# cubefs/cubefs

Measured on AMD Instinct MI355X. Metric: GiB/s encode+CRC throughput, RS(k+m) per stripe, 1/2/4/8 MI355X vs CPU, higher is better.
Workload: dtype u8; 1 GPU; RS(6+3) fused encode+frame, 8 MiB shards, 1024 stripes/GPU; codemode=EC6P3, stripes_per_gpu=1024, crc_included=True, block_len=65536

## Files before the change

### cubefs_amd/csrc/gfrs_kernels.hip

```cpp
#include "gfrs_internal.h"

#include <cstdio>
#include <cstdlib>
#include <type_traits>

namespace gfrs {

static int env_grid(const char *name, int dflt) {
  const char *v = getenv(name);
  if (!v) return dflt;
  int x = atoi(v);
  return x > 0 ? x : dflt;
}

typedef uint32_t u32x4 __attribute__((ext_vector_type(4)));

static bool nt_enabled() {
  static int v = -1;
  if (v < 0) {
    const char *e = getenv("GFRS_NT");
    v = e ? (atoi(e) != 0) : 0;
  }
  return v == 1;
}
// ... 532 lines not shown
                     hipStream_t s) {
  ShardAddr a{ptrs, 0, 0, nptr};
  rs_dispatch<false>(a, in_idx, k, out_idx, nout, tabs, shard_len, nstripes,
                     nullptr, s);
}

void launch_rs_apply_strided(uint64_t base, uint64_t stripe_stride,
                             const int32_t *in_idx, int k,
                             const int32_t *out_idx, int nout,
                             const uint8_t *tabs, size_t shard_len,
                             int nstripes, hipStream_t s) {
  ShardAddr a{nullptr, base, stripe_stride, 0};
  rs_dispatch<false>(a, in_idx, k, out_idx, nout, tabs, shard_len, nstripes,
                     nullptr, s);
}

void launch_rs_verify(const uint64_t *ptrs, int nptr, const int32_t *in_idx,
                      int k, const int32_t *out_idx, int nout,
                      const uint8_t *tabs, size_t shard_len, int nstripes,
                      uint32_t *fail, hipStream_t s) {
  ShardAddr a{ptrs, 0, 0, nptr};
  rs_dispatch<true>(a, in_idx, k, out_idx, nout, tabs, shard_len, nstripes,
                    fail, s);
}

void launch_rs_verify_strided(uint64_t base, uint64_t stripe_stride,
                              const int32_t *in_idx, int k,
                              const int32_t *out_idx, int nout,
                              const uint8_t *tabs, size_t shard_len,
                              int nstripes, uint32_t *fail, hipStream_t s) {
  ShardAddr a{nullptr, base, stripe_stride, 0};
  rs_dispatch<true>(a, in_idx, k, out_idx, nout, tabs, shard_len, nstripes,
                    fail, s);
}


__global__ void probe_perm_k(uint32_t *out) {
  if (threadIdx.x == 0) {
    out[0] = __builtin_amdgcn_perm(0x44332211u, 0x88776655u, 0x03020100u);
    out[1] = __builtin_amdgcn_perm(0x44332211u, 0x88776655u, 0x07060504u);
    out[2] = __builtin_amdgcn_perm(0xAABBCCDDu, 0x11223344u, 0x0B0A0908u);
    out[3] = __builtin_amdgcn_perm(0xAABBCCDDu, 0x11223344u, 0x0F0E0D0Cu);
    out[4] = __builtin_amdgcn_perm(0x80808080u, 0x7F7F7F7Fu, 0x0B0A0908u);
  }
}

static int g_perm0 = -1;

int probe_perm_device(void) {
  uint32_t *d = nullptr;
  uint32_t h[5] = {1, 1, 1, 1, 1};
  if (hipMalloc(&d, sizeof(h)) != hipSuccess) return -100;
  hipLaunchKernelGGL(probe_perm_k, dim3(1), dim3(64), 0, nullptr, d);
  if (hipMemcpy(h, d, sizeof(h), hipMemcpyDeviceToHost) != hipSuccess) {
    hipFree(d);
    return -100;
  }
  hipFree(d);
  const bool order_ok = (h[0] == 0x88776655u) && (h[1] == 0x44332211u);
  if (!order_ok) return -103;
  fprintf(stderr,
          "gfrs perm probe: sel8-11(lo=0x11223344,hi=0xAABBCCDD)=%08x "
          "sel12-15=%08x sel8-11(sign)=%08x\n", h[2], h[3], h[4]);
  g_perm0 = (h[2] == 0u) ? 1 : 0;
  return g_perm0;
}

static bool perm0_ok() {
  if (g_perm0 < 0) {
    int r = probe_perm_device();
    if (r < 0) g_perm0 = 0;
  }
  return g_perm0 == 1;
}


#define CRC_POLY 0xEDB88320u
#define CRC_LEN 4

__device__ uint32_t g_crc_tab4[8][256];
__device__ uint32_t g_shift4k[4][256];
__device__ uint32_t g_shift1k[4][256];
__device__ uint32_t g_shift8k[4][256];

__device__ uint32_t g_pow8[40];

GFRS_DEV int64_t i64min(int64_t a, int64_t b) { return a < b ? a : b; }

GFRS_DEV uint32_t gf2_mulmod_d(uint32_t a, uint32_t b) {
  uint32_t prod = 0;
#pragma unroll 8
  for (int i = 31; i >= 0; i--) {
    if ((a >> i) & 1) prod ^= b;
    b = (b & 1) ? (b >> 1) ^ CRC_POLY : (b >> 1);
  }
  return prod;
}

GFRS_DEV uint32_t x8n_d(uint64_t len) {
  uint32_t op = 0x80000000u;
  int j = 0;
  while (len) {
    if (len & 1) op = gf2_mulmod_d(op, g_pow8[j]);
    len >>= 1;
    j++;
  }
  return op;
}

constexpr int CRC_BLOCKT = 256;

GFRS_DEV uint32_t xor3(uint32_t a, uint32_t b, uint32_t c) {
  return __builtin_amdgcn_bitop3_b32(a, b, c, 0x96);
}

GFRS_DEV uint32_t crc16_reg(const uint4 q, const uint32_t (*tab)[256]) {
  uint32_t c = 0;
#pragma unroll
  for (int j = 0; j < 2; j++) {
    const uint32_t w0 = (j == 0 ? q.x : q.z) ^ c;
    const uint32_t w1 = (j == 0 ? q.y : q.w);
    c = xor3(xor3(tab[7][w0 & 0xFF], tab[6][(w0 >> 8) & 0xFF],
                  tab[5][(w0 >> 16) & 0xFF]),
             xor3(tab[4][w0 >> 24], tab[3][w1 & 0xFF],
                  tab[2][(w1 >> 8) & 0xFF]),
             tab[1][(w1 >> 16) & 0xFF] ^ tab[0][w1 >> 24]);
  }
  return c;
}

GFRS_DEV uint32_t shift4k(uint32_t c, const uint32_t (*stab)[256]) {
  return xor3(stab[0][c & 0xFF], stab[1][(c >> 8) & 0xFF],
              stab[2][(c >> 16) & 0xFF]) ^
         stab[3][c >> 24];
}

GFRS_DEV uint32_t crc_chunk(const uint8_t *p, int len,
                            const uint32_t (*tab)[256], uint8_t *dst) {
  uint32_t c = 0;
  int i = 0;
  for (; i + 4 <= len; i += 4) {
    const uint32_t w = *reinterpret_cast<const uint32_t *>(p + i);
    if (dst) *reinterpret_cast<uint32_t *>(dst + i) = w;
    c ^= w;
    c = tab[3][c & 0xFF] ^ tab[2][(c >> 8) & 0xFF] ^ tab[1][(c >> 16) & 0xFF] ^
        tab[0][c >> 24];
  }
  for (; i < len; i++) {
    if (dst) dst[i] = p[i];
    c = tab[0][(c ^ p[i]) & 0xFF] ^ (c >> 8);
  }
  return c;
}

GFRS_DEV uint32_t crc_chunk16(const uint8_t *p, int len,
                              const uint32_t (*tab)[256]) {
  uint32_t c = 0;
  int i = 0;
  for (; i + 16 <= len; i += 16) {
    const uint4 q = *reinterpret_cast<const uint4 *>(p + i);
#pragma unroll
    for (int j = 0; j < 2; j++) {
      const uint32_t w0 = (j == 0 ? q.x : q.z) ^ c;
      const uint32_t w1 = (j == 0 ? q.y : q.w);
      c = xor3(xor3(tab[7][w0 & 0xFF], tab[6][(w0 >> 8) & 0xFF],
                    tab[5][(w0 >> 16) & 0xFF]),
// ... 1071 lines not shown
              const uint8_t b = tailb[c2 * 16 + (p - t0)];
              pv ^= gfmul1_lin(ctab + size_t(r * k + c2) * 32, b);
            }
            fdst[p] = pv;
            part ^= gf2_mulmod_d(x8tab[rbi - 1 - p], tab[0][pv]);
          }
        }
#pragma unroll
        for (int sh = 32; sh > 0; sh >>= 1)
          part ^= __shfl_xor(part, sh, 64);
        if ((threadIdx.x & 63) == 0)
          red[(threadIdx.x >> 6) * 16 + k + r] ^= part;
      }
    }

    __syncthreads();
    {
      const int j = int(threadIdx.x);
      if (j < k + GM) {
        const uint32_t it =
            payload == payload_full
                ? it_full
                : gf2_mulmod_d(x8n_d(uint64_t(payload)), 0xFFFFFFFFu);
        const uint32_t crc =
            ~(it ^ red[j] ^ red[16 + j] ^ red[32 + j] ^ red[48 + j]);
        *reinterpret_cast<uint32_t *>(
            dst + (stripe * (k + GM) + j) * dst_stride + f * block_len) = crc;
      }
    }
    if (tiny_len && f == frames_per_shard - 1) {
      const int j = int(threadIdx.x);
      const int64_t tp0 = (f + 1) * payload_full;
      if (j < k) {
        const uint8_t *sp = sbase + size_t(j) * shard_len + tp0;
        for (int b = 0; b < tiny_len; b++) tinyb[j * 64 + b] = sp[b];
      }
      __syncthreads();
      if (j < k + GM) {
        uint8_t *tb =
            dst + (stripe * (k + GM) + j) * dst_stride + (f + 1) * block_len;
        uint32_t cr = 0;
        for (int b = 0; b < tiny_len; b++) {
          uint8_t x;
          if (j < k) {
            x = tinyb[j * 64 + b];
          } else {
            x = 0;
            for (int c2 = 0; c2 < k; c2++)
              x ^= gfmul1_lin(ctab + size_t((j - k) * k + c2) * 32,
                              tinyb[c2 * 64 + b]);
          }
          tb[CRC_LEN + b] = x;
          cr = tab[0][(cr ^ x) & 0xFF] ^ (cr >> 8);
        }
        *reinterpret_cast<uint32_t *>(tb) =
            ~(gf2_mulmod_d(x8n_d(uint64_t(tiny_len)), 0xFFFFFFFFu) ^ cr);
      }
    }
    __syncthreads();
  }
}



typedef uint32_t u32x3a __attribute__((ext_vector_type(3)));
struct AlLd {
  uint4 v[4];
  u32x3a e;
};

template <bool FULL>
GFRS_DEV AlLd al_load(const uint8_t *sp, int r, int P, int nfull, int q0) {
  AlLd o;
#pragma unroll
  for (int i = 0; i < 4; i++) {
    const int q = q0 + 64 * i;
    const bool lm = FULL ? (i > 0 || q > 0 || r < 3)
                         : (q <= nfull && 16 * q - 4 - 4 * r < P &&
                            16 * q + 12 - 4 * r > 0);
    o.v[i] = lm ? *reinterpret_cast<const uint4 *>(sp + 16 * q)
                : uint4{0, 0, 0, 0};
  }
  const int qe = q0 + 193;
  const bool em = (threadIdx.x & 63) == 63 && r > 0 &&
                  (FULL || (qe <= nfull && 16 * qe - 4 - 4 * r < P));
  o.e = em ? *reinterpret_cast<const u32x3a *>(sp + 16 * qe)
           : u32x3a{0, 0, 0};
  return o;
}

GFRS_DEV uint32_t al_shl1(uint32_t edge, uint32_t own) {
  return uint32_t(__builtin_amdgcn_update_dpp(int(edge), int(own),
                                              0x130 , 0xF,
                                              0xF, false));
}
GFRS_DEV uint32_t al_rol1(uint32_t v) {
  return uint32_t(__builtin_amdgcn_update_dpp(0, int(v),
                                              0x134 , 0xF,
                                              0xF, false));
}

GFRS_DEV uint32_t al_mulmod(uint32_t a, uint32_t b) {
  uint32_t prod = 0;
#pragma unroll
  for (int i = 31; i >= 0; i--) {
    const uint32_t ma = uint32_t(int32_t(a << (31 - i)) >> 31);
    prod ^= b & ma;
    const uint32_t mb = uint32_t(int32_t(b << 31) >> 31);
    b = (b >> 1) ^ (CRC_POLY & mb);
  }
  return prod;
}

GFRS_DEV uint32_t al_wave_xor(uint32_t x) {
  x ^= uint32_t(__builtin_amdgcn_update_dpp(0, int(x), 0xB1 , 0xF, 0xF, true));
  x ^= uint32_t(__builtin_amdgcn_update_dpp(0, int(x), 0x4E , 0xF, 0xF, true));
  x ^= uint32_t(__builtin_amdgcn_update_dpp(0, int(x),
                                            0x141 , 0xF,
                                            0xF, true));
  x ^= uint32_t(__builtin_amdgcn_update_dpp(0, int(x), 0x140 ,
                                            0xF, 0xF, true));
  return uint32_t(__builtin_amdgcn_readlane(int(x), 0) ^
                  __builtin_amdgcn_readlane(int(x), 16) ^
                  __builtin_amdgcn_readlane(int(x), 32) ^
                  __builtin_amdgcn_readlane(int(x), 48));
}

template <int R>
GFRS_DEV void al_rot(uint4 (&d)[4], const AlLd &c) {
#pragma unroll
  for (int i = 0; i < 4; i++) {
    const uint4 own = c.v[i];
    uint32_t n[3] = {0, 0, 0};
#pragma unroll
    for (int j = 0; j < R; j++) {
      const uint32_t ownj = j == 0 ? own.x : j == 1 ? own.y : own.z;
      uint32_t edge;
      if (i < 3) {
        const uint4 nx = c.v[i < 3 ? i + 1 : 3];
        edge = al_rol1(j == 0 ? nx.x : j == 1 ? nx.y : nx.z);
      } else {
        edge = j == 0 ? c.e.x : j == 1 ? c.e.y : c.e.z;
      }
      n[j] = al_shl1(edge, ownj);
    }
    d[i] = R == 0   ? own
           : R == 1 ? uint4{own.y, own.z, own.w, n[0]}
           : R == 2 ? uint4{own.z, own.w, n[0], n[1]}
                    : uint4{own.w, n[0], n[1], n[2]};
  }
}

template <int GM, int WPS, int SKEL = 0, int ST = 0, int C0 = 0>
__global__ __launch_bounds__(CRC_BLOCKT, WPS) void rs_encode_frame_al_k(
    uint8_t *__restrict__ dst, size_t dst_stride, uint64_t base,
    uint64_t stripe_stride, size_t shard_len, int k,
    const uint8_t *__restrict__ tabs , int64_t total_frames,
    int64_t frames_per_shard, int tiny_len ) {
  constexpr int64_t block_len = 65536;
  constexpr int payload_full = 65532;
  extern __shared__ __attribute__((aligned(16))) unsigned char smem[];
  uint32_t(*tab)[256] = reinterpret_cast<uint32_t(*)[256]>(smem);
  uint32_t(*stab)[256] = reinterpret_cast<uint32_t(*)[256]>(smem + 8192);
  uint32_t *red = reinterpret_cast<uint32_t *>(smem + 12288);
  uint32_t *x8tab = reinterpret_cast<uint32_t *>(smem + 12288 + EF_RED);
  uint8_t *tailb = smem + 12288 + EF_RED + 64;
  uint8_t *tinyb = smem + 12288 + EF_RED + 64 + 256;
  uint32_t *c0b =
      reinterpret_cast<uint32_t *>(smem + 12288 + EF_RED + 64 + 256 + 1024);
  uint8_t *ctab = smem + 12288 + EF_RED + 64 + 256 + 1024 + 256;
  for (int i = threadIdx.x; i < 2048; i += CRC_BLOCKT)
    (&tab[0][0])[i] = (&g_crc_tab4[0][0])[i];
  for (int i = threadIdx.x; i < 1024; i += CRC_BLOCKT)
    (&stab[0][0])[i] = (&g_shift1k[0][0])[i];
  for (int i = threadIdx.x; i < GM * k * 2; i += CRC_BLOCKT)
    reinterpret_cast<uint4 *>(ctab)[i] =
        reinterpret_cast<const uint4 *>(tabs)[i];
  if (threadIdx.x == 0) {
    uint32_t v = 0x80000000u;
    for (int j = 0; j < 16; j++) {
      x8tab[j] = v;
      v = gf2_mulmod_d(v, g_pow8[0]);
    }
  }
  const int tid = int(threadIdx.x);
  const int ql0 = (tid >> 6) * 256 + (tid & 63);
  constexpr uint32_t INV16K = 0x479933FCu;
  const uint32_t op_pA = x8n_d(uint64_t(65536 - 16 * (ql0 + 192 + 1)));
  const uint32_t op_pB = gf2_mulmod_d(op_pA, INV16K);
  const uint32_t op_pC = gf2_mulmod_d(op_pB, INV16K);
  const uint32_t op_pD = gf2_mulmod_d(op_pC, INV16K);
  const uint32_t it_full =
      gf2_mulmod_d(x8n_d(uint64_t(payload_full)), 0xFFFFFFFFu);
  __syncthreads();

  const int64_t fr0 = blockIdx.x, frS = gridDim.x;
  int64_t stripe = fr0 / frames_per_shard;
  int64_t f = fr0 - stripe * frames_per_shard;
  const int64_t dstripe = frS / frames_per_shard;
  const int64_t drem = frS - dstripe * frames_per_shard;
  AlLd nx = {};
  if (fr0 < total_frames) {
    const int64_t p0 = f * payload_full;
    const int r = int((3 * f + 3) & 3);
    const int P = int(i64min(payload_full, int64_t(shard_len) - p0));
    nx = al_load<false>(
        as_global(base + stripe * stripe_stride) + (p0 - 4 - 4 * r), r, P,
        (P + 4) >> 4, ql0);
  }
  for (int64_t fr = fr0; fr < total_frames; fr += frS) {
    int64_t stripe2 = stripe + dstripe, f2 = f + drem;
    if (f2 >= frames_per_shard) {
      f2 -= frames_per_shard;
      ++stripe2;
    }
    const int64_t p0 = f * payload_full;
    const int r = int((3 * f + 3) & 3);
    const int P = int(i64min(payload_full, int64_t(shard_len) - p0));
    const int T = P + 4;
    const int nfull = T >> 4;
    const int tb = T & 15;
    const int ntot = (T + 15) >> 4;
    const int64_t abase = p0 - 4 - 4 * r;
    const uint8_t *sbase = as_global(base + stripe * stripe_stride);

    for (int j = threadIdx.x; j < 64; j += CRC_BLOCKT) red[j] = 0;
    __syncthreads();

    auto passes = [&](auto fullc) {
    constexpr bool FULL = decltype(fullc)::value;
    uint4 acc[GM][4];
    for (int h = 0; h < 4; h++) {
      if (!FULL && 1024 * h >= ntot) break;
      const int qp = 1024 * h + ql0;
      const bool tail = !FULL && tb != 0 && (nfull >> 10) == h;
#pragma unroll
      for (int rr = 0; rr < GM; rr++)
#pragma unroll
        for (int i = 0; i < 4; i++) acc[rr][i] = uint4{0, 0, 0, 0};

      uint32_t op = h == 0   ? op_pA
                    : h == 1 ? op_pB
                    : h == 2 ? op_pC
                             : op_pD;
      if (!FULL) {
        int np = 0;
#pragma unroll
        for (int i = 0; i < 4; i++)
          if (qp + 64 * i < nfull) np = i + 1;
        const int end = np ? 16 * (qp + 64 * (np - 1) + 1) : 0;
        op = x8n_d(uint64_t(T - end));
      }

      for (int c = 0; c < k; c++) {
        const uint8_t *src = sbase + size_t(c) * shard_len;
        uint8_t *fdst =
            dst + (stripe * (k + GM) + c) * dst_stride + f * block_len;
        LinTab lt[GM];
        if (SKEL != 1)
#pragma unroll
          for (int rr = 0; rr < GM; rr++)
            lt[rr] = lintab_load(ctab, rr * k + c);
        const AlLd cur = nx;
        if (c + 1 < k)
          nx = al_load<FULL>(src + shard_len + abase, r, P, nfull, qp);
        uint4 d[4];
        switch (r) {
          case 0: al_rot<0>(d, cur); break;
          case 1: al_rot<1>(d, cur); break;
          case 2: al_rot<2>(d, cur); break;
          default: al_rot<3>(d, cur); break;
        }
        if (qp == 0) d[0].x = 0;
        uint32_t t = 0;
#pragma unroll
        for (int i = 0; i < 4; i++) {
          const int q = qp + 64 * i;
          if (FULL || q < nfull) {
            const uint4 v = d[i];
            if (SKEL != 1) {
#pragma unroll
              for (int dd = 0; dd < 4; dd++)
                gfmac4_lin_rows<GM>(acc, i, dd, (&v.x)[dd], lt);
            }
            if (i == 0 && q == 0) {
              if (C0 == 0) {
                *reinterpret_cast<u32x3a *>(fdst + 4) =
                    u32x3a{v.y, v.z, v.w};
              } else {
                c0b[c * 4 + 1] = v.y;
                c0b[c * 4 + 2] = v.z;
                c0b[c * 4 + 3] = v.w;
              }
            } else {
              fstore16<ST>(fdst + 16 * q, v);
            }
            if (SKEL != 1) t = shift4k(t, stab) ^ crc16_reg(v, tab);
          }
        }
        uint32_t part = al_mulmod(op, t);
        if (tail) {
          const int p = 16 * nfull + tid;
          if (p < T) {
            const uint8_t x = src[p0 + p - 4];
            fdst[p] = x;
            tailb[c * 16 + tid] = x;
            if (SKEL != 1)
              part ^= gf2_mulmod_d(x8tab[T - 1 - p], tab[0][x]);
          }
        }
        part = al_wave_xor(part);
        if ((tid & 63) == 0) red[(tid >> 6) * 16 + c] ^= part;
      }
      if (tail) __syncthreads();
      {
        if (FULL ? h < 3 : 1024 * (h + 1) < ntot) {
          nx = al_load<FULL>(sbase + abase, r, P, nfull, qp + 1024);
        } else if (fr + frS < total_frames) {
          const int64_t p02 = f2 * payload_full;
          const int r2 = int((3 * f2 + 3) & 3);
          const int P2 = int(i64min(payload_full, int64_t(shard_len) - p02));
          nx = al_load<false>(as_global(base + stripe2 * stripe_stride) +
                                  (p02 - 4 - 4 * r2),
                              r2, P2, (P2 + 4) >> 4, ql0);
        }
      }
#pragma unroll
      for (int rr = 0; rr < GM; rr++) {
        uint8_t *fdst =
            dst + (stripe * (k + GM) + k + rr) * dst_stride + f * block_len;
        uint32_t t = 0;
#pragma unroll
        for (int i = 0; i < 4; i++) {
          const int q = qp + 64 * i;
          if (FULL || q < nfull) {
            const uint4 v = acc[rr][i];
            if (i == 0 && q == 0) {
              if (C0 == 0) {
                *reinterpret_cast<u32x3a *>(fdst + 4) =
                    u32x3a{v.y, v.z, v.w};
              } else {
                c0b[(k + rr) * 4 + 1] = v.y;
                c0b[(k + rr) * 4 + 2] = v.z;
                c0b[(k + rr) * 4 + 3] = v.w;
              }
            } else {
              fstore16<ST>(fdst + 16 * q, v);
            }
            if (SKEL != 1) t = shift4k(t, stab) ^ crc16_reg(v, tab);
          }
        }
        uint32_t part = al_mulmod(op, t);
        if (SKEL != 1 && tail) {
          const int p = 16 * nfull + tid;
          if (p < T) {
            uint8_t pv = 0;
            for (int c2 = 0; c2 < k; c2++) {
              const uint8_t b = tailb[c2 * 16 + tid];
              pv ^= gfmul1_lin(ctab + size_t(rr * k + c2) * 32, b);
            }
            fdst[p] = pv;
            part ^= gf2_mulmod_d(x8tab[T - 1 - p], tab[0][pv]);
          }
        }
        part = al_wave_xor(part);
        if ((tid & 63) == 0) red[(tid >> 6) * 16 + k + rr] ^= part;
      }
    }
    };
    if (P == payload_full)
      passes(std::true_type{});
    else
      passes(std::false_type{});

    __syncthreads();
    {
      const int j = tid;
      if (j < k + GM) {
        const uint32_t it =
            P == payload_full
                ? it_full
                : gf2_mulmod_d(x8n_d(uint64_t(P)), 0xFFFFFFFFu);
        const uint32_t crc =
            ~(it ^ red[j] ^ red[16 + j] ^ red[32 + j] ^ red[48 + j]);
        uint8_t *fb0 =
            dst + (stripe * (k + GM) + j) * dst_stride + f * block_len;
        if (C0 == 1 && nfull > 0)
          *reinterpret_cast<uint4 *>(fb0) =
              uint4{crc, c0b[j * 4 + 1], c0b[j * 4 + 2], c0b[j * 4 + 3]};
        else
          *reinterpret_cast<uint32_t *>(fb0) = crc;
      }
    }
    if (tiny_len && f == frames_per_shard - 1) {
      const int j = tid;
      const int64_t tp0 = (f + 1) * payload_full;
      if (j < k) {
        const uint8_t *sp = sbase + size_t(j) * shard_len + tp0;
        for (int b = 0; b < tiny_len; b++) tinyb[j * 64 + b] = sp[b];
      }
      __syncthreads();
      if (j < k + GM) {
        uint8_t *tb2 =
            dst + (stripe * (k + GM) + j) * dst_stride + (f + 1) * block_len;
        uint32_t cr = 0;
        for (int b = 0; b < tiny_len; b++) {
          uint8_t x;
          if (j < k) {
            x = tinyb[j * 64 + b];
          } else {
            x = 0;
            for (int c2 = 0; c2 < k; c2++)
              x ^= gfmul1_lin(ctab + size_t((j - k) * k + c2) * 32,
                              tinyb[c2 * 64 + b]);
          }
          tb2[CRC_LEN + b] = x;
          cr = tab[0][(cr ^ x) & 0xFF] ^ (cr >> 8);
        }
        *reinterpret_cast<uint32_t *>(tb2) =
            ~(gf2_mulmod_d(x8n_d(uint64_t(tiny_len)), 0xFFFFFFFFu) ^ cr);
      }
    }
    __syncthreads();
    stripe = stripe2;
    f = f2;
  }
}




GFRS_DEV uint32_t crc_dw(uint32_t c, uint32_t w, const uint32_t (*tab)[256]) {
  c ^= w;
  return tab[3][c & 0xFF] ^ tab[2][(c >> 8) & 0xFF] ^
         tab[1][(c >> 16) & 0xFF] ^ tab[0][c >> 24];
}

GFRS_DEV uint32_t shift8k(uint32_t c, const uint32_t (*stab)[256]) {
  return xor3(stab[0][c & 0xFF], stab[1][(c >> 8) & 0xFF],
              stab[2][(c >> 16) & 0xFF]) ^
         stab[3][c >> 24];
}

GFRS_DEV uint32_t crc32_reg(const uint4 qa, const uint4 qb,
                            const uint32_t (*tab)[256]) {
  uint32_t c = 0;
#pragma unroll
  for (int j = 0; j < 4; j++) {
    const uint32_t w0 =
        (j == 0 ? qa.x : j == 1 ? qa.z : j == 2 ? qb.x : qb.z) ^ c;
    const uint32_t w1 = (j == 0 ? qa.y : j == 1 ? qa.w : j == 2 ? qb.y : qb.w);
    c = xor3(xor3(tab[7][w0 & 0xFF], tab[6][(w0 >> 8) & 0xFF],
                  tab[5][(w0 >> 16) & 0xFF]),
             xor3(tab[4][w0 >> 24], tab[3][w1 & 0xFF],
                  tab[2][(w1 >> 8) & 0xFF]),
             tab[1][(w1 >> 16) & 0xFF] ^ tab[0][w1 >> 24]);
  }
  return c;
}

typedef uint32_t u32x3_t __attribute__((ext_vector_type(3)));
template <int D0>
GFRS_DEV void rot_tail_load(uint4 &w2, const uint8_t *p) {
  if (D0 == 1) {
    w2.x = *reinterpret_cast<const uint32_t *>(p);
  } else if (D0 == 2) {
    const uint2 t = *reinterpret_cast<const uint2 *>(p);
    w2.x = t.x;
    w2.y = t.y;
  } else if (D0 == 3) {
    const u32x3_t t = *reinterpret_cast<const u32x3_t *>(p);
    w2.x = t.x;
    w2.y = t.y;
    w2.z = t.z;
  }
}

template <int D0>
GFRS_DEV void rot_pick(uint4 &h0, uint4 &h1, const uint4 w0, const uint4 w1,
                       const uint4 w2) {
  const uint32_t a[12] = {w0.x, w0.y, w0.z, w0.w, w1.x, w1.y,
                          w1.z, w1.w, w2.x, w2.y, w2.z, w2.w};
  h0 = uint4{a[D0], a[D0 + 1], a[D0 + 2], a[D0 + 3]};
  h1 = uint4{a[D0 + 4], a[D0 + 5], a[D0 + 6], a[D0 + 7]};
}

struct RotArgs {
  uint8_t *dst;
  const uint8_t *sbase;
  size_t dst_stride, shard_len;
  int64_t stripe, f, p0, payload, payload_eff;
  int k;
  const uint8_t *ctab;
  const uint32_t (*tab)[256];
// ... 1566 lines not shown
  const int64_t groups = (int64_t(nstripes) + 3) / 4;
  const int64_t cap = env_grid("GFRS_CRC_GRID", 16384);
  int grid = int(groups < cap ? groups : cap);
  if (grid < 1) grid = 1;
  const int ni = int((shard_len + 1023) / 1024);
  const int lds = 12288 + 64 + 1024 + m * k * 32;
  const uint8_t *ltabs = tabs;
#define GFRS_SM_GO(G, I)                                                  \
  hipLaunchKernelGGL((rs_encode_frame_small_k<G, I>), dim3(grid),         \
                     dim3(CRC_BLOCKT), lds, s, dst, dst_stride, base,     \
                     stripe_stride, shard_len, k, ltabs, nstripes)
#define GFRS_SM_NI(G)                                                     \
  switch (ni) {                                                           \
    case 1: GFRS_SM_GO(G, 1); break;                                      \
    case 2: GFRS_SM_GO(G, 2); break;                                      \
    case 3: GFRS_SM_GO(G, 3); break;                                      \
    default: GFRS_SM_GO(G, 4);                                            \
  }
#define GFRS_SM_GO3(G, I)                                                 \
  hipLaunchKernelGGL((rs_encode_frame_small_k<G, I, 3>), dim3(grid),      \
                     dim3(CRC_BLOCKT), lds, s, dst, dst_stride, base,     \
                     stripe_stride, shard_len, k, ltabs, nstripes)
#define GFRS_SM_NI8(G)                                                    \
  switch (ni) {                                                           \
    case 1: GFRS_SM_GO(G, 1); break;                                      \
    case 2: GFRS_SM_GO(G, 2); break;                                      \
    case 3: GFRS_SM_GO(G, 3); break;                                      \
    case 4: GFRS_SM_GO(G, 4); break;                                      \
    case 5: GFRS_SM_GO(G, 5); break;                                      \
    case 6: GFRS_SM_GO3(G, 6); break;                                     \
    case 7: GFRS_SM_GO3(G, 7); break;                                     \
    default: GFRS_SM_GO3(G, 8);                                           \
  }
  switch (m) {
    case 1: GFRS_SM_NI8(1); break;
    case 2: GFRS_SM_NI8(2); break;
    case 3: GFRS_SM_NI8(3); break;
    default: GFRS_SM_NI(4);
  }
#undef GFRS_SM_NI8
#undef GFRS_SM_GO3
#undef GFRS_SM_NI
#undef GFRS_SM_GO
}

constexpr bool kAlAuto = true;

void launch_rs_encode_frame(uint8_t *dst, size_t dst_stride, uint64_t base,
                            uint64_t stripe_stride, size_t shard_len, int k,
                            int m, const uint8_t *tabs, int nstripes,
                            hipStream_t s) {
  const int64_t fps = (int64_t(shard_len) + 65531) / 65532;
  const int64_t total = fps * nstripes;
  const int grid = fused_grid(total, fps);
  const uint8_t *ltabs = tabs;
  const int64_t tiny0 =
      fps >= 2 ? int64_t(shard_len) - (fps - 1) * 65532 : int64_t(0);
  const int tinyi = (tiny0 > 0 && tiny0 <= 64) ? int(tiny0) : 0;
  const int64_t fps2 = tinyi ? fps - 1 : fps;
  const int64_t total2 = fps2 * nstripes;
  const int grid2 = tinyi ? fused_grid(total2, fps2) : grid;
  static const int var_env = []() {
    const char *e = getenv("GFRS_EF");
    const int v = e ? atoi(e) : -1;
    switch (v) {
      case 13: case 14: case 23: case 24:
      case 72: case 73:
      case 74: case 75: case 76: case 77: case 78: case 79:
      case 86: case 87: case 96: case 97:
      case 103: case 104: case 113: case 114:
      case 142: case 152: case 162: return v;
      default: return -1;
    }
  }();
  const int var_old = shard_len >= (size_t(1) << 20) ? 76 : 87;
  const bool al_ok = ((uint64_t(reinterpret_cast<uintptr_t>(dst)) |
                       uint64_t(dst_stride) | base | stripe_stride |
                       uint64_t(shard_len)) & 15) == 0;
  const int var = var_env == 79 ? (al_ok ? 79 : var_old)
                  : var_env >= 0 ? var_env
                  : (kAlAuto && al_ok && var_old == 76) ? 79
                                                        : var_old;
  if (var == 79) {
    const int lds = 12288 + EF_RED + 64 + 256 + 1024 + 256 + m * k * 32;
#define GFRS_AL_GO(G, SK, C)                                              \
  hipLaunchKernelGGL((rs_encode_frame_al_k<G, 3, SK, 0, C>), dim3(grid2), \
                     dim3(CRC_BLOCKT), lds, s, dst, dst_stride, base,     \
                     stripe_stride, shard_len, k, ltabs, total2, fps2,    \
                     tinyi)
    static const int al_abl = []() {
      const char *e = getenv("GFRS_EF_ABL");
      return e ? atoi(e) : 0;
    }();
    static const int al_c0 = []() {
      const char *e = getenv("GFRS_EF_C0");
      return e ? atoi(e) : 0;
    }();
    if (m == 3 && var_env == 79 && al_abl == 4) { GFRS_AL_GO(3, 1, 0); return; }
    if (m == 3 && var_env == 79 && al_c0 == 1) { GFRS_AL_GO(3, 0, 1); return; }
    switch (m) {
      case 1: GFRS_AL_GO(1, 0, 0); break;
      case 2: GFRS_AL_GO(2, 0, 0); break;
      case 3: GFRS_AL_GO(3, 0, 0); break;
      default: GFRS_AL_GO(4, 0, 0);
    }
#undef GFRS_AL_GO
    return;
  }
  if (var == 103 || var == 104 || var == 113 || var == 114) {
    const int lds = 12288 + EF_RED + 128 + 512 + m * k * 32;
#define GFRS_ROT_GO(G, W, S)                                                hipLaunchKernelGGL((rs_encode_frame_rot_k<G, W, S>), dim3(grid),                             dim3(CRC_BLOCKT), lds, s, dst, dst_stride, base,                          stripe_stride, shard_len, k, ltabs, total, fps)
#define GFRS_ROT_SW(W, S)                                                   switch (m) {                                                                case 1: GFRS_ROT_GO(1, W, S); break;                                      case 2: GFRS_ROT_GO(2, W, S); break;                                      case 3: GFRS_ROT_GO(3, W, S); break;                                      default: GFRS_ROT_GO(4, W, S);                                          }
    if (var == 103) { GFRS_ROT_SW(3, 0) }
    else if (var == 104) { GFRS_ROT_SW(4, 0) }
    else if (var == 113) { GFRS_ROT_SW(3, 1) }
    else { GFRS_ROT_SW(4, 1) }
#undef GFRS_ROT_SW
#undef GFRS_ROT_GO
    return;
  }
  if (var == 72 || var == 73) {
    const int lds = 12288 + EF_RED + 64 + 256 + 1024 + m * k * 32;
#define GFRS_LO_GO(G, P)                                                    hipLaunchKernelGGL((rs_encode_frame_reg_k<G, 2, 0, 0, P>),                                   dim3(grid2), dim3(CRC_BLOCKT), lds, s, dst,                                dst_stride, base, stripe_stride, shard_len, k,                            ltabs, total2, fps2, tinyi)
#define GFRS_LO_SW(P)                                                       switch (m) {                                                                case 1: GFRS_LO_GO(1, P); break;                                          case 2: GFRS_LO_GO(2, P); break;                                          case 3: GFRS_LO_GO(3, P); break;                                          default: GFRS_LO_GO(4, P);                                              }
    if (var == 72) { GFRS_LO_SW(2) } else { GFRS_LO_SW(1) }
#undef GFRS_LO_SW
#undef GFRS_LO_GO
    return;
  }
  if (var == 86 || var == 87 || var == 96 || var == 97) {
    const int lds = 12288 + EF_RED + 64 + 256 + 1024 + m * k * 32;
#define GFRS_STP_GO(G, W, S)                                                hipLaunchKernelGGL((rs_encode_frame_reg_k<G, W, 0, 0, 1, S>),                                dim3(grid2), dim3(CRC_BLOCKT), lds, s, dst,                                dst_stride, base, stripe_stride, shard_len, k,                            ltabs, total2, fps2, tinyi)
#define GFRS_STP_SW(W, S)                                                   switch (m) {                                                                case 1: GFRS_STP_GO(1, W, S); break;                                      case 2: GFRS_STP_GO(2, W, S); break;                                      case 3: GFRS_STP_GO(3, W, S); break;                                      default: GFRS_STP_GO(4, W, S);                                          }
    if (var == 86) { GFRS_STP_SW(3, 1) }
    else if (var == 87) { GFRS_STP_SW(4, 1) }
    else if (var == 96) { GFRS_STP_SW(3, 2) }
    else { GFRS_STP_SW(4, 2) }
#undef GFRS_STP_SW
#undef GFRS_STP_GO
    return;
  }
  if (var == 77 && m == 3) {
    static const int map77 = []() {
      const char *e = getenv("GFRS_EF_MAP");
      return e ? atoi(e) : 0;
    }();
    if (map77 == 1 || map77 == 2) {
      const int lds = 12288 + EF_RED + 64 + 256 + 1024 + m * k * 32;
      if (map77 == 1)
        hipLaunchKernelGGL((rs_encode_frame_reg_k<3, 4, 1, 0, 1>),
                           dim3(grid2), dim3(CRC_BLOCKT), lds, s, dst,
                           dst_stride, base, stripe_stride, shard_len, k,
                           ltabs, total2, fps2, tinyi);
      else
        hipLaunchKernelGGL((rs_encode_frame_reg_k<3, 4, 2, 0, 1>),
                           dim3(grid2), dim3(CRC_BLOCKT), lds, s, dst,
                           dst_stride, base, stripe_stride, shard_len, k,
                           ltabs, total2, fps2, tinyi);
      return;
    }
  }
  if (var == 78) {
    const int lds = 12288 + EF_RED + 64 + 256 + 1024 + m * k * 32;
    switch (m) {
      case 1: hipLaunchKernelGGL((rs_encode_frame_reg_k<1, 3, 0, 0, 2>),
          dim3(grid2), dim3(CRC_BLOCKT), lds, s, dst, dst_stride, base,
          stripe_stride, shard_len, k, ltabs, total2, fps2, tinyi); break;
      case 2: hipLaunchKernelGGL((rs_encode_frame_reg_k<2, 3, 0, 0, 2>),
// ... 1003 lines not shown
      for (int i = 0; i < nf; i++) {
        const uint32_t fcv = __shfl(mine, i, 64);
        const int64_t plen = remain < payload_full ? remain : payload_full;
        if (f0 + i == 0) {
          crc = fcv;
        } else {
          const uint32_t op =
              plen == payload_full ? op_full : x8n_d(uint64_t(plen));
          crc = gf2_mulmod_d(op, crc) ^ fcv;
        }
        remain -= plen;
      }
    }
    const uint8_t *ftr = img + 32 + (raw_size + CRC_LEN * nframes);
    if (!(ftr[0] == 0xcc && ftr[1] == 0xef && ftr[2] == 0xcd &&
          ftr[3] == 0xab))
      status |= GFRS_SHARD_FTR_MAGIC;
    const uint32_t want_f = (uint32_t(ftr[4]) << 24) |
                            (uint32_t(ftr[5]) << 16) |
                            (uint32_t(ftr[6]) << 8) | uint32_t(ftr[7]);
    if (want_f != crc) status |= GFRS_SHARD_FTR_CRC;
  }
  gfrs_sresult r;
  r.status = status;
  r.crc = crc;
  r.bad_block = bb;
  r.bid = bid;
  r.vuid = vuid;
  r.size = size;
  if (lane == 0) results[j] = r;
}

void launch_shard_head_queue(uint64_t chunk, const gfrs_sjob *jobs,
                             const uint64_t *job_frame, const uint32_t *fcrc,
                             const int64_t *bad, gfrs_sresult *results,
                             int njobs, hipStream_t s) {
  if (njobs <= 0) return;
  const int wps = 4;
  const int blocks = (njobs + wps - 1) / wps;
  hipLaunchKernelGGL(shard_head_queue_k, dim3(blocks), dim3(wps * 64), 0, s,
                     chunk, jobs, job_frame, fcrc, bad, results, njobs);
}

int crc_device_init_current(void) {
  uint32_t tab[8][256];
  for (uint32_t i = 0; i < 256; i++) {
    uint32_t c = i;
    for (int j = 0; j < 8; j++) c = (c & 1) ? (c >> 1) ^ CRC_POLY : c >> 1;
    tab[0][i] = c;
  }
  for (int t = 1; t < 8; t++)
    for (int i = 0; i < 256; i++)
      tab[t][i] = tab[0][tab[t - 1][i] & 0xFF] ^ (tab[t - 1][i] >> 8);
  auto mulmod = [](uint32_t a, uint32_t b) {
    uint32_t prod = 0;
    for (int i = 31; i >= 0; i--) {
      if ((a >> i) & 1) prod ^= b;
      b = (b & 1) ? (b >> 1) ^ CRC_POLY : (b >> 1);
    }
    return prod;
  };
  uint32_t pow8[40];
  uint32_t p = 0x00800000u;
  for (int j = 0; j < 40; j++) {
    pow8[j] = p;
    p = mulmod(p, p);
  }
  uint32_t s4k[4][256];
  for (int j = 0; j < 4; j++)
    for (uint32_t b = 0; b < 256; b++)
      s4k[j][b] = mulmod(pow8[12], b << (8 * j));
  if (hipMemcpyToSymbol(HIP_SYMBOL(g_shift4k), s4k, sizeof(s4k)) != hipSuccess)
    return -100;
  for (int j = 0; j < 4; j++)
    for (uint32_t b = 0; b < 256; b++)
      s4k[j][b] = mulmod(pow8[10], b << (8 * j));
  if (hipMemcpyToSymbol(HIP_SYMBOL(g_shift1k), s4k, sizeof(s4k)) != hipSuccess)
    return -100;
  for (int j = 0; j < 4; j++)
    for (uint32_t b = 0; b < 256; b++)
      s4k[j][b] = mulmod(pow8[13], b << (8 * j));
  if (hipMemcpyToSymbol(HIP_SYMBOL(g_shift8k), s4k, sizeof(s4k)) != hipSuccess)
    return -100;
  if (hipMemcpyToSymbol(HIP_SYMBOL(g_crc_tab4), tab, sizeof(tab)) != hipSuccess)
    return -100;
  if (hipMemcpyToSymbol(HIP_SYMBOL(g_pow8), pow8, sizeof(pow8)) != hipSuccess)
    return -100;
  return 0;
}

void launch_crc_encode(uint8_t *dst, size_t dst_stride, const uint8_t *src,
                       size_t src_stride, int64_t n, int64_t block_len,
                       int nshards, hipStream_t s) {
  const int64_t payload = block_len - CRC_LEN;
  const int64_t fps = (n + payload - 1) / payload;
  crc_dispatch<0>(dst, dst_stride, src, src_stride, n, block_len, fps,
                  fps * nshards, nullptr, s);
}

void launch_crc_verify(const uint8_t *framed, size_t stride,
                       int64_t framed_len, int64_t block_len, int nshards,
                       int64_t *bad, hipStream_t s) {
  const int64_t fps = (framed_len + block_len - 1) / block_len;
  const int64_t n = framed_len - CRC_LEN * fps;
  crc_dispatch<1>(nullptr, 0, framed, stride, n, block_len, fps,
                  fps * nshards, bad, s);
}

void launch_crc_decode(uint8_t *dst, size_t dst_stride, const uint8_t *framed,
                       size_t src_stride, int64_t framed_len,
                       int64_t block_len, int nshards, int64_t *bad,
                       hipStream_t s) {
  const int64_t fps = (framed_len + block_len - 1) / block_len;
  const int64_t n = framed_len - CRC_LEN * fps;
  crc_dispatch<2>(dst, dst_stride, framed, src_stride, n, block_len, fps,
                  fps * nshards, bad, s);
}

}
```

Measured before the change: 1643 GiB/s.

## Chain per-thread CRC across passes via LDS running state and shift table

For full frames, each thread now carries its partial CRC across the four 16K passes. It stores the running value in an LDS array and advances it with a new 13K-shift table, instead of doing a carryless multiply per pass per shard. A single multiply-and-reduce per shard runs at the end. The per-pass rotation is also restructured into per-piece inlined functions with register pinning, and the tiny-frame loops are kept scalar. This trades more LDS use, which can lower occupancy, and extra LDS traffic for fewer al_mulmod and wave reductions.

```diff
diff --git a/cubefs_amd/csrc/gfrs_kernels.hip b/cubefs_amd/csrc/gfrs_kernels.hip
--- a/cubefs_amd/csrc/gfrs_kernels.hip
+++ b/cubefs_amd/csrc/gfrs_kernels.hip
@@ -638,6 +638,7 @@
 __device__ uint32_t g_shift4k[4][256];
 __device__ uint32_t g_shift1k[4][256];
 __device__ uint32_t g_shift8k[4][256];
+__device__ uint32_t g_shift13k[4][256];
 
 __device__ uint32_t g_pow8[40];
 
@@ -1875,7 +1876,7 @@
                 : uint4{0, 0, 0, 0};
   }
   const int qe = q0 + 193;
-  const bool em = (threadIdx.x & 63) == 63 && r > 0 &&
+  const bool em = (q0 & 63) == 63  && r > 0 &&
                   (FULL || (qe <= nfull && 16 * qe - 4 - 4 * r < P));
   o.e = em ? *reinterpret_cast<const u32x3a *>(sp + 16 * qe)
            : u32x3a{0, 0, 0};
@@ -1894,6 +1895,7 @@
 }
 
 GFRS_DEV uint32_t al_mulmod(uint32_t a, uint32_t b) {
+  asm volatile("" : "+v"(a));
   uint32_t prod = 0;
 #pragma unroll
   for (int i = 31; i >= 0; i--) {
@@ -1919,30 +1921,43 @@
                   __builtin_amdgcn_readlane(int(x), 48));
 }
 
-template <int R>
-GFRS_DEV void al_rot(uint4 (&d)[4], const AlLd &c) {
-#pragma unroll
-  for (int i = 0; i < 4; i++) {
-    const uint4 own = c.v[i];
-    uint32_t n[3] = {0, 0, 0};
-#pragma unroll
-    for (int j = 0; j < R; j++) {
-      const uint32_t ownj = j == 0 ? own.x : j == 1 ? own.y : own.z;
-      uint32_t edge;
-      if (i < 3) {
-        const uint4 nx = c.v[i < 3 ? i + 1 : 3];
-        edge = al_rol1(j == 0 ? nx.x : j == 1 ? nx.y : nx.z);
-      } else {
-        edge = j == 0 ? c.e.x : j == 1 ? c.e.y : c.e.z;
-      }
-      n[j] = al_shl1(edge, ownj);
-    }
-    d[i] = R == 0   ? own
-           : R == 1 ? uint4{own.y, own.z, own.w, n[0]}
-           : R == 2 ? uint4{own.z, own.w, n[0], n[1]}
-                    : uint4{own.w, n[0], n[1], n[2]};
-  }
-}
+template <int R, int I>
+GFRS_DEV uint4 al_rot1(const AlLd &c) {
+  const uint4 own = c.v[I];
+  uint32_t n[3] = {0, 0, 0};
+#pragma unroll
+  for (int j = 0; j < R; j++) {
+    const uint32_t ownj = j == 0 ? own.x : j == 1 ? own.y : own.z;
+    uint32_t edge;
+    if (I < 3) {
+      const uint4 nx = c.v[I < 3 ? I + 1 : 3];
+      edge = al_rol1(j == 0 ? nx.x : j == 1 ? nx.y : nx.z);
+    } else {
+      edge = j == 0 ? c.e.x : j == 1 ? c.e.y : c.e.z;
+    }
+    n[j] = al_shl1(edge, ownj);
+  }
+  return R == 0   ? own
+         : R == 1 ? uint4{own.y, own.z, own.w, n[0]}
+         : R == 2 ? uint4{own.z, own.w, n[0], n[1]}
+                  : uint4{own.w, n[0], n[1], n[2]};
+}
+
+template <int I>
+GFRS_DEV uint4 al_rot_piece(const AlLd &c, int r) {
+  switch (r) {
+    case 0: return al_rot1<0, I>(c);
+    case 1: return al_rot1<1, I>(c);
+    case 2: return al_rot1<2, I>(c);
+    default: return al_rot1<3, I>(c);
+  }
+}
+
+GFRS_DEV void al_pin(uint4 &v) {
+  asm volatile("" : "+v"(v.x), "+v"(v.y), "+v"(v.z), "+v"(v.w));
+}
+
+constexpr int AL_LDS_FIXED = 12288 + EF_RED + 64 + 256 + 1024 + 256 + 4096;
 
 template <int GM, int WPS, int SKEL = 0, int ST = 0, int C0 = 0>
 __global__ __launch_bounds__(CRC_BLOCKT, WPS) void rs_encode_frame_al_k(
@@ -1961,11 +1976,16 @@
   uint8_t *tinyb = smem + 12288 + EF_RED + 64 + 256;
   uint32_t *c0b =
       reinterpret_cast<uint32_t *>(smem + 12288 + EF_RED + 64 + 256 + 1024);
-  uint8_t *ctab = smem + 12288 + EF_RED + 64 + 256 + 1024 + 256;
+  uint32_t(*stab13)[256] = reinterpret_cast<uint32_t(*)[256]>(
+      smem + 12288 + EF_RED + 64 + 256 + 1024 + 256);
+  uint32_t *run0 = reinterpret_cast<uint32_t *>(smem + AL_LDS_FIXED);
+  uint8_t *ctab = smem + AL_LDS_FIXED + (k + GM + 1) * 1024;
   for (int i = threadIdx.x; i < 2048; i += CRC_BLOCKT)
     (&tab[0][0])[i] = (&g_crc_tab4[0][0])[i];
   for (int i = threadIdx.x; i < 1024; i += CRC_BLOCKT)
     (&stab[0][0])[i] = (&g_shift1k[0][0])[i];
+  for (int i = threadIdx.x; i < 1024; i += CRC_BLOCKT)
+    (&stab13[0][0])[i] = (&g_shift13k[0][0])[i];
   for (int i = threadIdx.x; i < GM * k * 2; i += CRC_BLOCKT)
     reinterpret_cast<uint4 *>(ctab)[i] =
         reinterpret_cast<const uint4 *>(tabs)[i];
@@ -1978,11 +1998,7 @@
   }
   const int tid = int(threadIdx.x);
   const int ql0 = (tid >> 6) * 256 + (tid & 63);
-  constexpr uint32_t INV16K = 0x479933FCu;
-  const uint32_t op_pA = x8n_d(uint64_t(65536 - 16 * (ql0 + 192 + 1)));
-  const uint32_t op_pB = gf2_mulmod_d(op_pA, INV16K);
-  const uint32_t op_pC = gf2_mulmod_d(op_pB, INV16K);
-  const uint32_t op_pD = gf2_mulmod_d(op_pC, INV16K);
+  run0[(k + GM) * 256 + tid] = x8n_d(uint64_t(16384 - 16 * (ql0 + 192 + 1)));
   const uint32_t it_full =
       gf2_mulmod_d(x8n_d(uint64_t(payload_full)), 0xFFFFFFFFu);
   __syncthreads();
@@ -2017,25 +2033,30 @@
     const int64_t abase = p0 - 4 - 4 * r;
     const uint8_t *sbase = as_global(base + stripe * stripe_stride);
 
-    for (int j = threadIdx.x; j < 64; j += CRC_BLOCKT) red[j] = 0;
+    int tidf = int(threadIdx.x);
+    asm volatile("" : "+v"(tidf));
+    const int tid = tidf;
+    const int ql0 = (tid >> 6) * 256 + (tid & 63);
+    uint32_t *run = run0 + tid;
+
+    if (tid < 64) red[tid] = 0;
     __syncthreads();
 
     auto passes = [&](auto fullc) {
     constexpr bool FULL = decltype(fullc)::value;
     uint4 acc[GM][4];
+#pragma unroll 1
     for (int h = 0; h < 4; h++) {
       if (!FULL && 1024 * h >= ntot) break;
-      const int qp = 1024 * h + ql0;
+      int qp = 1024 * h + ql0;
+      if (!FULL) asm volatile("" : "+v"(qp));
       const bool tail = !FULL && tb != 0 && (nfull >> 10) == h;
 #pragma unroll
       for (int rr = 0; rr < GM; rr++)
 #pragma unroll
         for (int i = 0; i < 4; i++) acc[rr][i] = uint4{0, 0, 0, 0};
 
-      uint32_t op = h == 0   ? op_pA
-                    : h == 1 ? op_pB
-                    : h == 2 ? op_pC
-                             : op_pD;
+      uint32_t op = 0;
       if (!FULL) {
         int np = 0;
 #pragma unroll
@@ -2057,20 +2078,15 @@
         const AlLd cur = nx;
         if (c + 1 < k)
           nx = al_load<FULL>(src + shard_len + abase, r, P, nfull, qp);
-        uint4 d[4];
-        switch (r) {
-          case 0: al_rot<0>(d, cur); break;
-          case 1: al_rot<1>(d, cur); break;
-          case 2: al_rot<2>(d, cur); break;
-          default: al_rot<3>(d, cur); break;
-        }
-        if (qp == 0) d[0].x = 0;
         uint32_t t = 0;
-#pragma unroll
-        for (int i = 0; i < 4; i++) {
+        if (FULL && SKEL != 1) t = shift4k(h ? run[c * 256] : 0u, stab13);
+        auto piece = [&](auto ic) {
+          constexpr int i = decltype(ic)::value;
+          uint4 v = al_rot_piece<i>(cur, r);
+          al_pin(v);
+          if (i == 0 && qp == 0) v.x = 0;
           const int q = qp + 64 * i;
           if (FULL || q < nfull) {
-            const uint4 v = d[i];
             if (SKEL != 1) {
 #pragma unroll
               for (int dd = 0; dd < 4; dd++)
@@ -2088,8 +2104,17 @@
             } else {
               fstore16<ST>(fdst + 16 * q, v);
             }
-            if (SKEL != 1) t = shift4k(t, stab) ^ crc16_reg(v, tab);
-          }
+            if (SKEL != 1)
+              t = (FULL && i == 0 ? t : shift4k(t, stab)) ^ crc16_reg(v, tab);
+          }
+        };
+        piece(std::integral_constant<int, 0>{});
+        piece(std::integral_constant<int, 1>{});
+        piece(std::integral_constant<int, 2>{});
+        piece(std::integral_constant<int, 3>{});
+        if (FULL) {
+          if (SKEL != 1) run[c * 256] = t;
+          continue;
         }
         uint32_t part = al_mulmod(op, t);
         if (tail) {
@@ -2123,6 +2148,8 @@
         uint8_t *fdst =
             dst + (stripe * (k + GM) + k + rr) * dst_stride + f * block_len;
         uint32_t t = 0;
+        if (FULL && SKEL != 1)
+          t = shift4k(h ? run[(k + rr) * 256] : 0u, stab13);
 #pragma unroll
         for (int i = 0; i < 4; i++) {
           const int q = qp + 64 * i;
@@ -2140,8 +2167,13 @@
             } else {
               fstore16<ST>(fdst + 16 * q, v);
             }
-            if (SKEL != 1) t = shift4k(t, stab) ^ crc16_reg(v, tab);
-          }
+            if (SKEL != 1)
+              t = (FULL && i == 0 ? t : shift4k(t, stab)) ^ crc16_reg(v, tab);
+          }
+        }
+        if (FULL) {
+          if (SKEL != 1) run[(k + rr) * 256] = t;
+          continue;
         }
         uint32_t part = al_mulmod(op, t);
         if (SKEL != 1 && tail) {
@@ -2158,6 +2190,13 @@
         }
         part = al_wave_xor(part);
         if ((tid & 63) == 0) red[(tid >> 6) * 16 + k + rr] ^= part;
+      }
+    }
+    if (FULL && SKEL != 1) {
+      const uint32_t op_pD = run[(k + GM) * 256];
+      for (int j = 0; j < k + GM; j++) {
+        const uint32_t part = al_wave_xor(al_mulmod(op_pD, run[j * 256]));
+        if ((tid & 63) == 0) red[(tid >> 6) * 16 + j] ^= part;
       }
     }
     };
@@ -2190,6 +2229,7 @@
       const int64_t tp0 = (f + 1) * payload_full;
       if (j < k) {
         const uint8_t *sp = sbase + size_t(j) * shard_len + tp0;
+#pragma clang loop vectorize(disable) unroll(disable)
         for (int b = 0; b < tiny_len; b++) tinyb[j * 64 + b] = sp[b];
       }
       __syncthreads();
@@ -2197,12 +2237,14 @@
         uint8_t *tb2 =
             dst + (stripe * (k + GM) + j) * dst_stride + (f + 1) * block_len;
         uint32_t cr = 0;
+#pragma clang loop vectorize(disable) unroll(disable)
         for (int b = 0; b < tiny_len; b++) {
           uint8_t x;
           if (j < k) {
             x = tinyb[j * 64 + b];
           } else {
             x = 0;
+#pragma clang loop vectorize(disable) unroll(disable)
             for (int c2 = 0; c2 < k; c2++)
               x ^= gfmul1_lin(ctab + size_t((j - k) * k + c2) * 32,
                               tinyb[c2 * 64 + b]);
@@ -3935,8 +3977,9 @@
                   : (kAlAuto && al_ok && var_old == 76) ? 79
                                                         : var_old;
   if (var == 79) {
-    const int lds = 12288 + EF_RED + 64 + 256 + 1024 + 256 + m * k * 32;
-#define GFRS_AL_GO(G, SK, C)                                              \
+    const int lds =
+        AL_LDS_FIXED + (k + (m < 4 ? m : 4) + 1) * 1024 + m * k * 32;
+#define GFRS_AL_GO(G, SK, C)                                             \
   hipLaunchKernelGGL((rs_encode_frame_al_k<G, 3, SK, 0, C>), dim3(grid2), \
                      dim3(CRC_BLOCKT), lds, s, dst, dst_stride, base,     \
                      stripe_stride, shard_len, k, ltabs, total2, fps2,    \
@@ -5106,6 +5149,12 @@
       s4k[j][b] = mulmod(pow8[13], b << (8 * j));
   if (hipMemcpyToSymbol(HIP_SYMBOL(g_shift8k), s4k, sizeof(s4k)) != hipSuccess)
     return -100;
+  const uint32_t x13k = mulmod(mulmod(pow8[13], pow8[12]), pow8[10]);
+  for (int j = 0; j < 4; j++)
+    for (uint32_t b = 0; b < 256; b++)
+      s4k[j][b] = mulmod(x13k, b << (8 * j));
+  if (hipMemcpyToSymbol(HIP_SYMBOL(g_shift13k), s4k, sizeof(s4k)) != hipSuccess)
+    return -100;
   if (hipMemcpyToSymbol(HIP_SYMBOL(g_crc_tab4), tab, sizeof(tab)) != hipSuccess)
     return -100;
   if (hipMemcpyToSymbol(HIP_SYMBOL(g_pow8), pow8, sizeof(pow8)) != hipSuccess)
```

New measurement: 1906 GiB/s, median of 6. 1.16x the previous value.
